# forfd8960/audio-flow-rs

Measured on NVIDIA B200. Metric: audio_seconds_per_second, higher is better.
Workload: dtype f32

## Files before the change

audio-flow-rs_b200/audioflow/__init__.py:

```python
from __future__ import annotations

import ctypes as C
import os
from dataclasses import dataclass
from enum import IntEnum

import numpy as np

_HERE = os.path.dirname(os.path.abspath(__file__))
LIB_PATH = os.environ.get("AF_GPU_LIB") or os.path.join(os.path.dirname(_HERE), "lib", "libaudioflow_gpu.so")

AF_OK, AF_ERR_INVALID, AF_ERR_RESAMPLING_FAILED, AF_ERR_CUDA, AF_ERR_NO_DEVICE, AF_ERR_CAPACITY = range(6)
AF_FMT_F32, AF_FMT_I16 = 0, 1
AF_MEM_DEVICE, AF_MEM_HOST = 0, 1


class AudioError(Exception):
    """src-tauri/src/error.rs:96-111; only ResamplingFailed arises on this path."""


class ResamplingFailed(AudioError):
    def __init__(self, msg: str):
        super().__init__("Resampling failed: " + msg)
        self.msg = msg
# ... 109 lines not shown
        "af_batch_run_host": (C.c_int, [vp, C.POINTER(OutputsC)]),
        "af_pipeline_run": (C.c_int, [vp, C.POINTER(StreamDescC), sz, C.POINTER(OutputsC)]),
        "af_set_kernel_variant": (C.c_int, [C.c_char_p]),
        "af_vad_segments": (C.c_int, [vp, C.c_uint64, vp, sz, vp, C.c_uint32, vp, vp]),
        "af_vad_gate": (C.c_int, [vp, C.c_uint64, vp, C.c_uint64, C.c_uint32, vp, C.c_uint32, vp, C.c_uint32, vp, sz,
                                  C.POINTER(GateOutputsC), vp]),
        "af_current_device": (C.c_int, []), "af_set_stream": (C.c_int, [vp]), "af_init_multi": (C.c_int, [C.c_int]),
        "af_comm_unique_id": (C.c_int, [u8p]), "af_comm_init_rank": (C.c_int, [C.c_int, C.c_int, u8p]),
        "af_comm_size": (C.c_int, []), "af_comm_shutdown": (C.c_int, []),
        "af_shard_partition": (C.c_int, [C.POINTER(StreamDescC), sz, C.c_int, szp]),
        "af_sharded_batch_create": (C.c_int, [vp, C.POINTER(StreamDescC), sz, C.c_int, C.POINTER(vp)]),
        "af_sharded_batch_destroy": (None, [vp]),
        "af_sharded_batch_shard": (C.c_int, [vp, C.c_int, szp, szp, C.POINTER(C.c_int)]),
        "af_sharded_batch_local": (vp, [vp, C.c_int]),
        "af_sharded_batch_run": (C.c_int, [vp, C.POINTER(ShardedOutputsC), C.c_int, C.c_int]),
        "af_sharded_batch_wait": (C.c_int, [vp]), "af_sharded_batch_join": (C.c_int, [vp]),
        "af_sharded_batch_gathered": (C.c_int, [vp, C.c_int, C.POINTER(vp), C.POINTER(C.c_uint64), C.POINTER(C.c_uint64),
                                                C.POINTER(C.c_uint32)]),
        "af_sharded_batch_gathered_host": (C.c_int, [vp, C.c_int, u8p, C.c_uint64]),
        "af_sharded_batch_gather_ms": (C.c_int, [vp, C.c_int, fp]),
        "af_sharded_batch_run_host": (C.c_int, [vp, C.POINTER(OutputsC)]),
        "af_debug_vad_energy_threshold": (C.c_float, [C.c_float]),
        "af_debug_resample_plan": (sz, [C.c_uint32, C.c_uint32, sz, fp, sz, C.POINTER(C.c_int)]),
        "af_session_create": (C.c_int, [vp, sz, C.c_uint32, C.c_uint16, C.c_uint16, C.c_uint32, C.POINTER(vp)]),
        "af_session_destroy": (None, [vp]),
        "af_session_push": (C.c_int, [vp, vp, C.c_uint64, C.c_uint32, C.c_int, C.POINTER(OutputsC),
                                      C.POINTER(C.c_uint32), C.POINTER(C.c_uint32), C.POINTER(C.c_uint32)]),
        "af_session_reset": (C.c_int, [vp]),
        "af_session_enable_levels": (C.c_int, [vp, C.c_int]),
        "af_session_levels": (C.c_int, [vp, fp, fp, u8p]),
        "af_session_enable_wire": (C.c_int, [vp, C.POINTER(WireConfigC)]),
        "af_session_wire": (C.c_int, [vp, C.POINTER(vp), C.POINTER(C.c_uint64), C.POINTER(vp), C.POINTER(C.c_uint64),
                                      C.POINTER(WireTickC), C.POINTER(C.c_uint64)]),
        "af_ring_create": (C.c_int, [sz, C.POINTER(vp)]), "af_ring_destroy": (None, [vp]),
        "af_ring_capacity": (sz, [vp]), "af_ring_write": (sz, [vp, fp, sz]),
        "af_ring_read": (C.c_int, [vp, fp, sz, szp]), "af_ring_available": (sz, [vp]), "af_ring_clear": (None, [vp]),
        "af_session_push_rings": (C.c_int, [vp, C.POINTER(vp), C.c_uint32, C.POINTER(OutputsC),
                                            C.POINTER(C.c_uint32), C.POINTER(C.c_uint32), C.POINTER(C.c_uint32)]),
        "af_session_push_streams": (C.c_int, [vp, vp, C.c_uint64, C.POINTER(C.c_uint32), u8p, C.c_int, C.POINTER(OutputsC),
                                              C.POINTER(C.c_uint32), C.POINTER(C.c_uint32), C.POINTER(C.c_uint32)]),
        "af_session_reset_streams": (C.c_int, [vp, C.POINTER(C.c_uint32), sz]),
        "af_session_push_rings_available": (C.c_int, [vp, C.POINTER(vp), C.c_uint32, u8p, C.POINTER(OutputsC),
                                                      C.POINTER(C.c_uint32), C.POINTER(C.c_uint32), C.POINTER(C.c_uint32)]),
        "af_session_wire_first_frames": (C.c_int, [vp, C.POINTER(C.c_uint64)]),
        "af_session_create_formats": (C.c_int, [vp, sz, C.POINTER(StreamFormatC), sz, C.POINTER(C.c_uint32), C.c_uint16,
                                                C.POINTER(vp)]),
# ... 216 lines not shown
    def energy_db(self) -> float: return float(load_library().af_vad_energy_db(self._h))
    def is_speaking(self) -> bool: return bool(load_library().af_vad_is_speaking(self._h))
    def speech_frame_count(self) -> int: return int(load_library().af_vad_speech_frame_count(self._h))
    def smoothed_energy(self) -> float: return float(load_library().af_vad_smoothed_energy(self._h))


def pcm16_encode(samples) -> np.ndarray:
    x = _f32(samples)
    out = np.empty(len(x), np.int16)
    _check(load_library().af_pcm16_encode(_fp(x), len(x), out.ctypes.data_as(C.POINTER(C.c_int16))))
    return out


def pcm16_base64(samples) -> bytes:
    L = load_library()
    x = _f32(samples)
    cap = int(L.af_pcm16_base64_len(len(x)))
    buf = C.create_string_buffer(max(cap, 1))
    n = C.c_size_t(0)
    _check(L.af_pcm16_base64(_fp(x), len(x), buf, cap, C.byref(n)))
    return buf.raw[:n.value]


def pipeline_config(n_mels: int = 80, vad: VadConfig | None = None, vad_enable: bool = True, vad_frame_len: int = 0,
                    vad_hop: int = 0, write_pcm: bool = True, log10: bool = False, f_min: float = 0.0,
                    f_max: float = 8000.0, log_floor: float = 1e-10, pcm16: bool = False) -> PipelineConfigC:
    c = PipelineConfigC()
    load_library().af_pipeline_config_default(C.byref(c))
    c.n_mels = n_mels
    c.f_min, c.f_max, c.log_floor, c.log10 = f_min, f_max, log_floor, int(log10)
    c.vad_enable = int(vad_enable)
    if vad is not None:
        c.vad = vad._c()
    c.vad_frame_len, c.vad_hop = vad_frame_len, vad_hop
    c.write_pcm = int(write_pcm)
    c.pcm16 = int(pcm16)
    return c


class Pipeline:
    def __init__(self, cfg: PipelineConfigC | None = None):
        self.cfg = cfg if cfg is not None else pipeline_config()
        h = C.c_void_p()
        _check(load_library().af_pipeline_create(C.byref(self.cfg), C.byref(h)))
        self._h = h

    def __del__(self):
        if getattr(self, "_h", None) and _lib is not None:
            _lib.af_pipeline_destroy(self._h)
            self._h = None

    def batch(self, descs, mem: int) -> "Batch":
        return Batch(self, descs, mem)

    def run_host(self, streams):
        arrays, descs = [], []
        for (x, rate, ch) in streams:
            if x.dtype == np.int16:
                a, fmt = np.ascontiguousarray(x), AF_FMT_I16
            else:
                a, fmt = _f32(x), AF_FMT_F32
            arrays.append(a)
            descs.append((a.ctypes.data, a.size, rate, ch, fmt))
        b = Batch(self, descs, AF_MEM_HOST)
        out = b.alloc_host_outputs()
        b.run_host(out)
        return b.split(out)


def _desc_array(descs):
    arr = (StreamDescC * max(len(descs), 1))()
    for i, (ptr, n_samples, rate, ch, fmt) in enumerate(descs):
        arr[i] = StreamDescC(ptr or None, n_samples, rate, ch, fmt)
# ... 399 lines not shown
```

audio-flow-rs_b200/csrc/af_common.cuh:

```cuda
#pragma once
#include <cstddef>
#include <cstdint>
#include <cuda_runtime.h>

namespace af {

constexpr int OUT_RATE = 16000;
constexpr int WIN = 400;
constexpr int HOP = 160;
constexpr int NFFT = 512;
constexpr int NBIN = NFFT / 2 + 1;
constexpr int MAX_MELS = 128;

constexpr int RS_CHUNK = 128;
constexpr int RS_POLY = 8;

constexpr int SF = 32;
constexpr int STEP_SAMPLES = SF * HOP;
constexpr int CARRY = WIN - HOP;
constexpr int YLEN = STEP_SAMPLES + CARRY;
constexpr int N_STAGE = 2;
constexpr int MAX_PARTS = 4;
__host__ __device__ constexpr int part_end(int parts, int k)
{
// ... 172 lines not shown
    int state;
    unsigned long long silence_frames;
    unsigned long long speech_frames;
};

struct FusedParams {
    const StreamDev *streams;
    const TileDev *tiles;
    uint32_t n_tiles;
    const FftTables *fft;
    const MelTables *mel;
    float *pcm;   uint64_t pcm_stride;
    float *logmel; uint64_t logmel_stride;
    float *energy; uint64_t energy_stride;
    uint32_t n_mels;
    uint32_t do_energy;
    float log_floor;
    float log_scale;
    uint32_t use_stage;
    uint32_t layout;
    uint32_t quarters;
    float neg_zero;
    uint32_t per_p, per_q;
};

}
```

audio-flow-rs_b200/csrc/af_fused.cu:

```cuda
#include <atomic>
#include <type_traits>

#ifdef AF_FUSED_SPLIT_TU
#define af_fused_kernel af_fused_split_kernel
#define g_pipe_stats g_pipe_stats_split
#endif

#include "af_device.cuh"
#include "af_launch.h"

namespace af {

constexpr int AF_MAX_GPUS_INTERNAL = 16;

struct alignas(16) RsTile {
    uint32_t stream_idx, tile;
    int tile_k;
    uint32_t tile_rem;
    uint32_t n_steps, tile_end, n_frames, parts;
    StreamDev stream;
    uint32_t inc_k, inc_rem;
};
static_assert(sizeof(RsTile) == 112 && offsetof(RsTile, stream) == 32, "RsTile mirrors the head and the tail of TileDev");
static_assert(offsetof(TileDev, sdesc) % 16 == 0 && sizeof(TileDev) - offsetof(TileDev, sdesc) == 80 && offsetof(TileDev, parts) == 28 &&
              offsetof(TileDev, inc_k) == offsetof(TileDev, sdesc) + sizeof(StreamDev), "TileDev layout the cp.async prefetch relies on");

struct __align__(128) FusedSmem {
    unsigned char stage[N_STAGE][STAGE_BYTES];
    float ybuf[2][YBUF_FLOATS];
    float scr[FFT_WARPS * SCR_FLOATS_PER_WARP];
    float pbuf[2][PBUF_FLOATS];
    uint32_t tmem_base;
// ... 776 lines not shown
    {                                                                                               \
        float w_[16];                                                                               \
        tmem_ld16(tq + 16u * (i), w_);                                                              \
        const float4 xa = pa[i], xb = pb[i], xc = pc[i], xd = pd[i];                                \
        tmem_wait_ld(w_);                                                                           \
        const float4 wa = make_float4(w_[0], w_[1], w_[2], w_[3]), wb = make_float4(w_[4], w_[5], w_[6], w_[7]);       \
        const float4 wc = make_float4(w_[8], w_[9], w_[10], w_[11]), wd = make_float4(w_[12], w_[13], w_[14], w_[15]); \
        AF_MEL_FMA16()                                                                              \
    }
#define AF_MEL_CHAIN(STEP)                                                                          \
    switch (c4) {                                                                                   \
    case 8: STEP(7)                                                                                 \
    case 7: STEP(6)                                                                                 \
    case 6: STEP(5)                                                                                 \
    case 5: STEP(4)                                                                                 \
    case 4: STEP(3)                                                                                 \
    case 3: STEP(2)                                                                                 \
    case 2: STEP(1)                                                                                 \
    case 1: STEP(0)                                                                                 \
    default: break;                                                                                 \
    }

template <bool FAST_LOG, bool VEC>
__device__ __forceinline__ void role_mel_run(FusedSmem &sm, const FusedParams &P, int mw, int lane)
{
    const uint32_t M = P.n_mels;
    const float log_mul = P.log_scale, log_floor = P.log_floor;
    const int q0 = sm.mel.quad_begin[mw], q1 = sm.mel.quad_begin[mw + 1];
    const int fr = pb_frame(lane);
    const uint32_t tm = sm.tmem_base + ((uint32_t)(32 * ((threadIdx.x >> 5) & 3)) << 16);
    AF_STATS_DECL
    for (uint32_t it = 0;; ++it) {
        const int b = (int)(it & 1u);
        AF_WAIT(&sm.p_full[b], (it >> 1) & 1u, 0);
        const StepInfo info = sm.pinfo[it & 3u];
        const int n_valid = info.n_valid & 0xff;
        if (M && info.lm_dst && n_valid > 0) {
            const bool valid = fr < n_valid;
            float *dst = info.lm_dst + (uint32_t)fr * M + 4 * q0;
            const char *prow = reinterpret_cast<const char *>(sm.pbuf[b] + lane * PB_ROW);
            const uint4 *qtab = reinterpret_cast<const uint4 *>(&sm.mel.quad[q0]);
            for (int qd = q0; qd < q1; ++qd, qtab += 2, dst += 4) {
                const uint4 d0q = qtab[0], d1q = qtab[1];
                const float4 *pa = reinterpret_cast<const float4 *>(prow + d0q.x);
                const float4 *pb = reinterpret_cast<const float4 *>(prow + d0q.y);
                const float4 *pc = reinterpret_cast<const float4 *>(prow + d0q.z);
                const float4 *pd = reinterpret_cast<const float4 *>(prow + d0q.w);
                int c4 = (int)d1q.x;
                float a0 = 0.0f, a1 = 0.0f, b0 = 0.0f, b1 = 0.0f, c0 = 0.0f, c1 = 0.0f, d0 = 0.0f, d1 = 0.0f;
                if (d1q.z != MEL_NO_TMEM) {
                    const uint32_t tq = tm + d1q.z;
                    AF_MEL_CHAIN(AF_MEL_STEP_T)
                } else {
                    const float4 *w4 = reinterpret_cast<const float4 *>(reinterpret_cast<const char *>(sm.mel.w) + d1q.y);
#pragma unroll 1
                    for (; c4 > 8; --c4) AF_MEL_STEP_S(c4 - 1)
                    AF_MEL_CHAIN(AF_MEL_STEP_S)
                }
                float o[4];
                if (FAST_LOG) {
                    o[0] = lg2_ftz(fmaxf(a0 + a1, log_floor)) * log_mul;
                    o[1] = lg2_ftz(fmaxf(b0 + b1, log_floor)) * log_mul;
                    o[2] = lg2_ftz(fmaxf(c0 + c1, log_floor)) * log_mul;
                    o[3] = lg2_ftz(fmaxf(d0 + d1, log_floor)) * log_mul;
                } else {
                    o[0] = __log2f(fmaxf(a0 + a1, log_floor)) * log_mul;
                    o[1] = __log2f(fmaxf(b0 + b1, log_floor)) * log_mul;
                    o[2] = __log2f(fmaxf(c0 + c1, log_floor)) * log_mul;
                    o[3] = __log2f(fmaxf(d0 + d1, log_floor)) * log_mul;
                }
                if (valid) {
                    if (VEC) __stcs(reinterpret_cast<float4 *>(dst), make_float4(o[0], o[1], o[2], o[3]));
                    else {
#pragma unroll
                        for (int u = 0; u < 4; ++u)
                            if (4 * qd + u < (int)M) dst[u] = o[u];
                    }
                }
            }
        }
        warp_arrive(&sm.p_empty[b], lane);
        if (info.n_valid & STEP_LAST) break;
    }
    AF_STATS_FLUSH(1, lane);
}
#undef AF_MEL_CHAIN
#undef AF_MEL_STEP_T
#undef AF_MEL_STEP_S
#undef AF_MEL_FMA16

__device__ __forceinline__ void role_mel(FusedSmem &sm, const FusedParams &P, int mw, int lane)
{
    const bool fast_log = P.log_floor >= 1.17549435e-38f;
    const bool vec = (P.n_mels & 3u) == 0 && (P.logmel_stride & 3ull) == 0 && ((reinterpret_cast<uintptr_t>(P.logmel) & 15) == 0);
    if (fast_log && vec) role_mel_run<true, true>(sm, P, mw, lane);
    else if (vec) role_mel_run<false, true>(sm, P, mw, lane);
    else role_mel_run<false, false>(sm, P, mw, lane);
}

template <bool QUARTERS>
__device__ __forceinline__ void role_vad(FusedSmem &sm, const FusedParams &P, int lane, int vidx)
{
    const bool chains = P.do_energy && P.energy;
    if (vidx != 0 && !chains) return;
    AF_STATS_DECL
    uint32_t tile_f = blockIdx.x, g_f = 0, it_f = 0, steps_f = 0;
    int h_f = 0;
    bool fill_live = vidx == 0 && tile_f < P.n_tiles;
    FillDesc d_next{};
    auto fetch_desc = [&]() {
        const uint4 *src = reinterpret_cast<const uint4 *>(&P.tiles[tile_f].fill[2 * g_f + h_f]);
        const uint4 a = __ldg(src), b = __ldg(src + 1);
        d_next.src = reinterpret_cast<const char *>(((unsigned long long)a.y << 32) | a.x);
        d_next.bytes = a.z; d_next.lo = a.w; d_next.hi = b.x; d_next.interior = b.y;
    };
    auto tile_pairs = [&]() { return QUARTERS ? P.tiles[tile_f].n_steps * (P.tiles[tile_f].parts >> 1) : P.tiles[tile_f].n_steps; };
    if (lane == 0 && fill_live) { steps_f = tile_pairs(); fetch_desc(); }
    auto issue_next = [&](bool blocking) {
        if (!fill_live) return;
        if (blocking) { AF_WAIT(&sm.stage_empty[h_f], (it_f & 1u) ^ 1u, 0); }
// ... 426 lines not shown
```

audio-flow-rs_b200/csrc/af_plan.cpp:

```cpp
#include "af_plan.h"

#include <algorithm>
#include <cmath>
#include <cstring>
#include <limits>
#include <numeric>

namespace af {

void RsRecurrence::init(uint32_t in, uint32_t out)
{
    in_rate = in; out_rate = out;
    passthrough = (in == out);
    const uint32_t g = std::gcd(in, out);
    p = in / g; q = out / g;
    const double ratio = (double)out / (double)in;
    t = 1.0 / ratio;
    end_idx = (long)RS_CHUNK - (RS_POLY + 1) - (long)std::ceil(t);
    exact = (q & (q - 1)) == 0 && q <= (1u << 20) && t == (double)p / (double)q;
    last_index = -(double)(RS_POLY / 2);
    chunks = 0; n_out = 0;
}

uint32_t RsRecurrence::step(std::vector<float> *frac)
// ... 103 lines not shown
        cost[qd] = 24u * c4 + 40u;
        total += cost[qd];
    }
    t->n_w = (uint16_t)(16 * off16); t->n_mels = (uint16_t)n_mels;
    uint32_t q = 0, acc = 0;
    t->quad_begin[0] = 0;
    for (int j = 1; j < MEL_WARPS; ++j) {
        const uint32_t target = (uint32_t)(((uint64_t)total * (uint64_t)j) / MEL_WARPS);
        while (q < n_quads && acc + cost[q] / 2 < target) acc += cost[q++];
        t->quad_begin[j] = (uint16_t)q;
    }
    t->quad_begin[MEL_WARPS] = (uint16_t)n_quads;
    uint32_t next_col[4] = {TM_MEL0, TM_MEL0, TM_MEL0, TM_MEL0};
    for (int j = 0; j < MEL_WARPS; ++j) {
        uint32_t &col = next_col[j & 3];
        for (uint32_t qd = t->quad_begin[j]; qd < t->quad_begin[j + 1]; ++qd) {
            const uint32_t need = 16u * t->quad[qd].c4;
            if (t->quad[qd].c4 <= 8 && col + need <= TMEM_COLS) { t->quad[qd].tcol = col; col += need; }
        }
    }
    return true;
}

static inline float bits_to_f32(uint32_t b) { float f; std::memcpy(&f, &b, 4); return f; }

float vad_energy_threshold(float threshold_db)
{
    auto speech = [&](float e) { return 20.0f * log10f(e) > threshold_db; };
    const uint32_t inf_bits = 0x7f800000u;
    if (!speech(bits_to_f32(inf_bits))) return std::numeric_limits<float>::quiet_NaN();
    uint32_t lo = 1, hi = inf_bits;
    if (speech(bits_to_f32(lo))) return bits_to_f32(lo);
    while (hi - lo > 1) {
        const uint32_t mid = lo + (hi - lo) / 2;
        if (speech(bits_to_f32(mid))) hi = mid; else lo = mid;
    }
    return bits_to_f32(hi);
}

}
```

audio-flow-rs_b200/csrc/af_plan.h:

```cpp
#pragma once
#include <cstdint>
#include <vector>

#include "af_common.cuh"

namespace af {

struct RsRecurrence {
    uint32_t in_rate = 0, out_rate = 0;
    uint32_t p = 1, q = 1;
    double t = 1.0;
    long end_idx = 0;
    bool passthrough = false;
    bool exact = false;
    double last_index = -4.0;
    uint64_t chunks = 0;
    uint64_t n_out = 0;

    void init(uint32_t in, uint32_t out);
    uint32_t step(std::vector<float> *frac);
    uint32_t mode() const { return passthrough ? RS_PASSTHROUGH : (exact ? RS_EXACT : RS_TABLE); }
};

uint64_t rs_exact_count(const RsRecurrence &r, uint64_t chunks);

void build_fft_tables(FftTables *t);
bool build_mel_tables(uint32_t n_mels, float f_min, float f_max, MelTables *t);
float vad_energy_threshold(float threshold_db);

}
```

audio-flow-rs_b200/csrc/af_runtime.cu:

```cuda
#include <algorithm>
#include <cmath>
#include <cstdlib>
#include <cstring>

#include "af_internal.h"

using namespace af;
using namespace afrt;

namespace afrt {

namespace {
thread_local std::string g_err;
std::atomic<uint64_t> g_launches{0};
Context *const g_ctxs = new Context[MAX_DEV];
std::mutex g_init_mu;
std::atomic<int> g_default_dev{-1};
thread_local int t_dev = -1;
std::string g_variant = "auto";
}

int fail(int code, const char *fmt, ...)
{
    char buf[512];
    va_list ap;
    va_start(ap, fmt);
    vsnprintf(buf, sizeof(buf), fmt, ap);
    va_end(ap);
// ... 662 lines not shown
    cudaStream_t st = cuda_stream ? (cudaStream_t)cuda_stream : cur_ctx().stream;
    GateJob J{};
    J.pcm = out->pcm ? pcm : nullptr; J.pcm_stride = pcm_stride;
    J.logmel = out->logmel ? logmel : nullptr; J.logmel_stride = logmel_stride;
    J.n_mels = n_mels; J.hop = hop; J.n_out = n_out;
    J.seg = seg; J.seg_cap = seg_cap; J.n_seg = n_seg;
    J.off = out->seg_offset; J.total = out->n_frames;
    J.out_pcm = out->pcm; J.out_pcm_stride = out->pcm_stride;
    J.out_lm = out->logmel; J.out_lm_stride = out->logmel_stride;
    J.n_streams = (uint32_t)n_streams;
    AF_CUDA(launch_vad_gate(J, st));
    count_launch((J.out_pcm || J.out_lm) ? 2 : 1);
    if (!cuda_stream) AF_CUDA(cudaStreamSynchronize(st));
    return AF_OK;
}

}

struct af_pipeline {
    af_pipeline_config cfg;
    VadParams vad_prm;
    MelTables h_mel;
    DevBuf<MelTables> d_mel[MAX_DEV];
    std::mutex mu;
};

namespace {
MelTables *pipe_mel(af_pipeline *p)
{
    if (!p->cfg.n_mels) return nullptr;
    const int dev = cur_device();
    std::lock_guard<std::mutex> lk(p->mu);
    if (!p->d_mel[dev].get()) {
        cudaError_t e = p->d_mel[dev].alloc(1);
        if (e == cudaSuccess) e = cudaMemcpy(p->d_mel[dev].get(), &p->h_mel, sizeof(MelTables), cudaMemcpyHostToDevice);
        if (e != cudaSuccess) {
            p->d_mel[dev].reset();
            fail(AF_ERR_CUDA, "mel tables: %s", cudaGetErrorString(e));
        }
    }
    return p->d_mel[dev].get();
}
}

namespace {

struct HostStream {
    af_stream_desc desc;
    uint32_t n_in, n_out, n_frames, n_vad_frames, mode, p, q;
    std::shared_ptr<FracTable> table;
// ... 95 lines not shown
int run_sub(af_batch *b, SubBatch &sb, float *pcm, uint64_t pcm_stride, float *logmel, uint64_t logmel_stride,
            uint8_t *vad, uint64_t vad_stride, float *energy, uint64_t energy_stride, VadState *vad_final,
            cudaStream_t st)
{
    const af_pipeline_config &cfg = b->pipe->cfg;
    const bool stft_vad = cfg.vad_enable && cfg.vad_frame_len == 0;
    const bool custom_vad = cfg.vad_enable && cfg.vad_frame_len != 0;
    if (!sb.h_tiles.empty()) {
        FusedParams P{};
        P.streams = sb.d_streams.get(); P.tiles = sb.d_tiles.get(); P.n_tiles = (uint32_t)sb.h_tiles.size();
        P.fft = cur_ctx().d_fft.get(); P.mel = b->d_mel;
        P.pcm = pcm; P.pcm_stride = pcm_stride;
        P.logmel = cfg.n_mels ? logmel : nullptr; P.logmel_stride = logmel_stride;
        P.energy = stft_vad ? energy : nullptr; P.energy_stride = energy_stride;
        P.n_mels = (cfg.n_mels && logmel) ? cfg.n_mels : 0;
        P.do_energy = stft_vad ? 1 : 0;
        P.log_floor = cfg.log_floor;
        P.log_scale = cfg.log10 ? 0.30102999566398120f : 0.69314718055994531f;
        P.use_stage = kernel_variant() == "sync" ? 0u : 1u;
        P.layout = fused_layout(stft_vad);
        P.quarters = sb.quarters ? 1u : 0u;
        P.neg_zero = -0.0f;
        P.per_p = sb.per_p; P.per_q = sb.per_q;
        const int n_ctas = (int)std::min<size_t>(sb.h_tiles.size(), (size_t)cur_ctx().sm_count);
        AF_CUDA(launch_fused(P, n_ctas, st, sb.split));
        count_launch();
    }
    if (custom_vad) {
        EnergyJob ej{};
        ej.y = pcm; ej.y_stride = pcm_stride; ej.n_frames = sb.d_nvad.get(); ej.n_frames_all = (uint32_t)b->max_vad;
        ej.frame_len = cfg.vad_frame_len; ej.hop = cfg.vad_hop; ej.energy = energy; ej.energy_stride = energy_stride;
        ej.n_streams = (uint32_t)sb.count;
        AF_CUDA(launch_frame_energy(ej, st));
        count_launch();
    }
    if (cfg.vad_enable) {
        ScanJob sj{};
        sj.energy = energy; sj.energy_stride = energy_stride; sj.n_frames = sb.d_nvad.get(); sj.n_frames_all = 0;
        sj.states = vad; sj.states_stride = vad_stride; sj.state_io = nullptr; sj.final_out = vad_final;
        sj.prm = b->pipe->vad_prm; sj.n_streams = (uint32_t)sb.count;
        if (b->max_vad > 16384 && b->max_vad < 0x40000000ull) {
            AF_CUDA(sb.d_scan.grow(sb.count * scan_scratch_words((uint32_t)b->max_vad)));
            sj.max_frames = (uint32_t)b->max_vad; sj.scratch = sb.d_scan.get();
        }
        AF_CUDA(launch_vad_scan(sj, st));
        count_launch();
// ... 19 lines not shown
    cfg->log10 = 0;
    cfg->vad_enable = 1;
    af_vad_config_default(&cfg->vad);
    cfg->vad_frame_len = 0; cfg->vad_hop = 0;
    cfg->write_pcm = 1;
    cfg->pcm16 = 0;
}

AF_API int af_pipeline_create(const af_pipeline_config *cfg, af_pipeline **out)
{
    if (!out) return fail(AF_ERR_INVALID, "null out pointer");
    int rc = require_ctx();
    if (rc) return rc;
    af_pipeline_config c;
    if (cfg) c = *cfg; else af_pipeline_config_default(&c);
    if (c.n_mels > MAX_MELS) return fail(AF_ERR_INVALID, "n_mels %u > %d", c.n_mels, MAX_MELS);
    if (c.vad_enable && c.vad_frame_len != 0 && c.vad_hop == 0) return fail(AF_ERR_INVALID, "vad_hop must be positive");
    if (c.n_mels && !(c.f_max > c.f_min && c.f_min >= 0.0f)) return fail(AF_ERR_INVALID, "bad mel band [%g, %g]", c.f_min, c.f_max);
    af_pipeline *p = new af_pipeline;
    p->cfg = c;
    p->vad_prm = make_vad_params(c.vad);
    if (c.n_mels) {
        if (!build_mel_tables(c.n_mels, c.f_min, c.f_max, &p->h_mel)) { delete p; return fail(AF_ERR_INVALID, "mel table construction failed"); }
        if (!pipe_mel(p)) { delete p; return AF_ERR_CUDA; }
    }
    *out = p;
    return AF_OK;
}

AF_API void af_pipeline_destroy(af_pipeline *p)
{
    if (!p) return;
    for (int d = 0; d < MAX_DEV; ++d)
        if (p->d_mel[d].get() && device_ctx(d)) { DevScope scope_(d); p->d_mel[d].reset(); }
    delete p;
}

AF_API void af_batch_destroy(af_batch *b)
{
    if (!b) return;
    DevScope scope_(b->device);
    cudaDeviceSynchronize();
    for (auto &s : b->slots)
        if (s.st) cudaStreamDestroy(s.st);
    delete b;
}
// ... 277 lines not shown
            if (o->energy)
                AF_CUDA(cudaMemcpy2DAsync(o->energy + r0 * o->energy_stride, o->energy_stride * sizeof(float), sl.d_energy.get(),
                                          b->energy_stride * sizeof(float), b->max_vad * sizeof(float), sb.count,
                                          cudaMemcpyDeviceToHost, st));
        }
        if (cfg.vad_enable && o->vad_final)
            AF_CUDA(cudaMemcpyAsync(o->vad_final + r0, sl.d_final.get(), sb.count * sizeof(VadState), cudaMemcpyDeviceToHost, st));
    }
    for (auto &sl : b->slots) AF_CUDA(cudaStreamSynchronize(sl.st));
    return AF_OK;
}

AF_API int af_pipeline_run(af_pipeline *p, const af_stream_desc *streams, size_t n_streams, const af_outputs *out)
{
    af_batch *b = nullptr;
    int rc = af_batch_create(p, streams, n_streams, AF_MEM_HOST, &b);
    if (rc) return rc;
    rc = af_batch_run_host(b, out);
    af_batch_destroy(b);
    return rc;
}

AF_API float af_debug_vad_energy_threshold(float threshold_db) { return vad_energy_threshold(threshold_db); }

AF_API size_t af_debug_resample_plan(uint32_t input_rate, uint32_t output_rate, size_t n_chunks, float *frac, size_t cap,
                                     int *mode)
{
    RsRecurrence r;
    r.init(input_rate, output_rate);
    if (mode) *mode = (int)r.mode();
    if (r.passthrough || r.end_idx <= 0) return 0;
    std::vector<float> f;
    for (size_t c = 0; c < n_chunks; ++c) r.step(&f);
    for (size_t i = 0; i < f.size() && i < cap; ++i) frac[i] = f[i];
    return f.size();
}

}

struct af_session {
    af_pipeline *pipe = nullptr;
    int device = -1;
    MelTables *d_mel = nullptr;
    size_t S = 0;
    struct Format { uint32_t rate, channels, max_tick_frames; };
    std::vector<Format> fmts;
// ... 449 lines not shown
        AF_CUDA(cudaMemcpy2DAsync(o->pcm, o->pcm_stride * sizeof(float), pcm_rows, pcm_rows_stride * sizeof(float),
                                  (size_t)max_ny * sizeof(float), S, cudaMemcpyDeviceToHost, st));
    if (s->levels) {
        AF_CUDA(launch_peak(ycur + one.y_keep, s->y_stride, one.n_y, (uint32_t)S, s->lv.d_peak.get(), st, tab));
        count_launch();
    }

    if (maxT) {
        if (s->packed) {
            FusedParams P{};
            P.streams = s->d_ptab[y_next].get(); P.tiles = s->d_ptiles[y_next].get(); P.n_tiles = s->pk_n;
            const uint64_t vrows = s->pk_rows;
            P.fft = cur_ctx().d_fft.get(); P.mel = s->d_mel;
            P.pcm = nullptr; P.pcm_stride = 0;
            P.logmel = lm; P.logmel_stride = lm_stride * vrows;
            P.energy = cfg.vad_enable ? s->d_energy.get() : nullptr; P.energy_stride = s->energy_stride * vrows;
            P.n_mels = lm ? cfg.n_mels : 0;
            P.do_energy = cfg.vad_enable ? 1 : 0;
            P.log_floor = cfg.log_floor;
            P.log_scale = cfg.log10 ? 0.30102999566398120f : 0.69314718055994531f;
            P.use_stage = kernel_variant() == "sync" ? 0u : 1u;
            P.layout = fused_layout(P.do_energy != 0);
            P.neg_zero = -0.0f;
            if (P.n_mels || P.do_energy) {
                AF_CUDA(launch_fused(P, (int)std::min<size_t>(P.n_tiles, (size_t)cur_ctx().sm_count), st));
                count_launch(2);
            }
        } else {
            EnergyJob ej{};
            ej.y = ycur; ej.y_stride = s->y_stride; ej.n_frames = d_T; ej.n_frames_all = maxT;
            ej.frame_len = s->frame_len; ej.hop = s->hop; ej.energy = s->d_energy.get(); ej.energy_stride = s->energy_stride;
            ej.n_streams = (uint32_t)S;
            AF_CUDA(launch_frame_energy(ej, st));
            count_launch();
        }
        if (cfg.vad_enable) {
            ScanJob sj{};
            sj.energy = s->d_energy.get(); sj.energy_stride = s->energy_stride; sj.n_frames = d_T; sj.n_frames_all = maxT;
            sj.states = states; sj.states_stride = st_stride; sj.state_io = s->d_vad.get();
            sj.final_out = mem == AF_MEM_DEVICE ? reinterpret_cast<VadState *>(o->vad_final) : nullptr;
            sj.prm = s->pipe->vad_prm; sj.n_streams = (uint32_t)S;
            AF_CUDA(launch_vad_scan(sj, st));
            count_launch();
        }
        if (mem == AF_MEM_DEVICE && lm && lm != o->logmel)
            AF_CUDA(cudaMemcpy2DAsync(o->logmel, o->logmel_stride * sizeof(float), lm, lm_stride * sizeof(float),
// ... 373 lines not shown
```

include/audioflow_gpu.h:

```cpp
#ifndef AUDIOFLOW_GPU_H
#define AUDIOFLOW_GPU_H

#include <stddef.h>
#include <stdint.h>

#ifdef __cplusplus
extern "C" {
#endif

#if defined(__GNUC__)
#define AF_API __attribute__((visibility("default")))
#else
#define AF_API
#endif

typedef enum af_status {
    AF_OK = 0,
    AF_ERR_INVALID = 1,
    AF_ERR_RESAMPLING_FAILED = 2,
    AF_ERR_CUDA = 3,
    AF_ERR_NO_DEVICE = 4,
    AF_ERR_CAPACITY = 5
} af_status;

// ... 152 lines not shown
AF_API int af_shard_partition(const af_stream_desc *streams, size_t n_streams, int n_shards, size_t *first);

typedef struct af_sharded_batch af_sharded_batch;
typedef struct af_sharded_outputs {
    af_outputs shard[AF_MAX_GPUS];
} af_sharded_outputs;
AF_API int af_sharded_batch_create(af_pipeline *p, const af_stream_desc *streams, size_t n_streams, int mem,
                                   af_sharded_batch **out);
AF_API void af_sharded_batch_destroy(af_sharded_batch *b);
AF_API int af_sharded_batch_shard(const af_sharded_batch *b, int rank, size_t *first, size_t *count, int *device);
AF_API af_batch *af_sharded_batch_local(af_sharded_batch *b, int rank);
AF_API int af_sharded_batch_run(af_sharded_batch *b, const af_sharded_outputs *out, int gather, int async);
AF_API int af_sharded_batch_wait(af_sharded_batch *b);
AF_API int af_sharded_batch_join(af_sharded_batch *b);
AF_API int af_sharded_batch_gathered(af_sharded_batch *b, int rank, const uint8_t **states, uint64_t *row_stride,
                                     uint64_t *rows_per_rank, uint32_t *n_vad_frames);
AF_API int af_sharded_batch_gathered_host(af_sharded_batch *b, int rank, uint8_t *states, uint64_t stride);
AF_API int af_sharded_batch_gather_ms(af_sharded_batch *b, int rank, float *ms);
AF_API int af_sharded_batch_run_host(af_sharded_batch *b, const af_outputs *out);

AF_API float af_debug_vad_energy_threshold(float threshold_db);
AF_API size_t af_debug_resample_plan(uint32_t input_rate, uint32_t output_rate, size_t n_chunks, float *frac,
                                     size_t cap, int *mode);

typedef struct af_session af_session;
AF_API int af_session_create(af_pipeline *p, size_t n_streams, uint32_t sample_rate, uint16_t channels,
                             uint16_t format, uint32_t max_tick_samples, af_session **out);
AF_API void af_session_destroy(af_session *s);
AF_API int af_session_push(af_session *s, const void *data, uint64_t in_stride, uint32_t n_samples, int mem,
                           const af_outputs *out, uint32_t *n_pcm, uint32_t *n_feat, uint32_t *n_vad);
AF_API int af_session_reset(af_session *s);

AF_API int af_session_enable_levels(af_session *s, int enable);
AF_API int af_session_levels(const af_session *s, float *level_db, float *peak, uint8_t *is_speech);

typedef struct af_wire_config {
    uint32_t gate;
    uint32_t pcm16;
    uint32_t base64;
    int32_t mem;
} af_wire_config;
typedef struct af_wire_tick {
    uint32_t n_samples, n_chars, continued;
    uint16_t started, ended;
    uint8_t in_speech, pad[3];
} af_wire_tick;
// ... 39 lines not shown
```

Measured before the change: 13.51 million.

## Specialize mel filterbank for common configs with generated unrolled FMA walks

```diff
diff --git a/audio-flow-rs_b200/audioflow/__init__.py b/audio-flow-rs_b200/audioflow/__init__.py
--- a/audio-flow-rs_b200/audioflow/__init__.py
+++ b/audio-flow-rs_b200/audioflow/__init__.py
@@ -155,6 +155,8 @@
         "af_sharded_batch_run_host": (C.c_int, [vp, C.POINTER(OutputsC)]),
         "af_debug_vad_energy_threshold": (C.c_float, [C.c_float]),
         "af_debug_resample_plan": (sz, [C.c_uint32, C.c_uint32, sz, fp, sz, C.POINTER(C.c_int)]),
+        "af_debug_mel_bank": (C.c_int, [C.c_uint32, C.c_float, C.c_float, fp, fp, C.POINTER(C.c_uint32)]),
+        "af_debug_pipeline_mel_bank": (C.c_int, [vp]),
         "af_session_create": (C.c_int, [vp, sz, C.c_uint32, C.c_uint16, C.c_uint16, C.c_uint32, C.POINTER(vp)]),
         "af_session_destroy": (None, [vp]),
         "af_session_push": (C.c_int, [vp, vp, C.c_uint64, C.c_uint32, C.c_int, C.POINTER(OutputsC),
@@ -417,6 +419,18 @@
     return buf.raw[:n.value]
 
 
+def mel_bank(n_mels: int, f_min: float = 0.0, f_max: float = 8000.0) -> dict:
+    L = load_library()
+    plan = np.zeros((n_mels, 257), np.float32)
+    comp = np.full((n_mels, 257), np.nan, np.float32)
+    wb = (C.c_uint32 * 5)(*([0xFFFFFFFF] * 5))
+    bank = L.af_debug_mel_bank(n_mels, f_min, f_max, _fp(plan), _fp(comp), wb)
+    if bank < 0:
+        raise ValueError(f"no mel filterbank for n_mels={n_mels}, [{f_min}, {f_max}] Hz")
+    has = wb[0] != 0xFFFFFFFF
+    return {"bank": bank, "plan": plan, "compiled": comp if has else None, "warp_bands": list(wb) if has else None}
+
+
 def pipeline_config(n_mels: int = 80, vad: VadConfig | None = None, vad_enable: bool = True, vad_frame_len: int = 0,
                     vad_hop: int = 0, write_pcm: bool = True, log10: bool = False, f_min: float = 0.0,
                     f_max: float = 8000.0, log_floor: float = 1e-10, pcm16: bool = False) -> PipelineConfigC:
@@ -444,6 +458,10 @@
         if getattr(self, "_h", None) and _lib is not None:
             _lib.af_pipeline_destroy(self._h)
             self._h = None
+
+    @property
+    def mel_bank(self) -> int:
+        return int(load_library().af_debug_pipeline_mel_bank(self._h))
 
     def batch(self, descs, mem: int) -> "Batch":
         return Batch(self, descs, mem)
diff --git a/audio-flow-rs_b200/csrc/af_common.cuh b/audio-flow-rs_b200/csrc/af_common.cuh
--- a/audio-flow-rs_b200/csrc/af_common.cuh
+++ b/audio-flow-rs_b200/csrc/af_common.cuh
@@ -218,6 +218,7 @@
     uint32_t quarters;
     float neg_zero;
     uint32_t per_p, per_q;
-};
-
-}
+    uint32_t mel_bank;
+};
+
+}
diff --git a/audio-flow-rs_b200/csrc/af_fused.cu b/audio-flow-rs_b200/csrc/af_fused.cu
--- a/audio-flow-rs_b200/csrc/af_fused.cu
+++ b/audio-flow-rs_b200/csrc/af_fused.cu
@@ -8,6 +8,7 @@
 
 #include "af_device.cuh"
 #include "af_launch.h"
+#include "af_mel_banks.h"
 
 namespace af {
 
@@ -830,6 +831,32 @@
     }
 
 template <bool FAST_LOG, bool VEC>
+__device__ __forceinline__ void mel_out4(float *dst, int m0, uint32_t M, bool valid, float log_floor, float log_mul, float s0,
+                                         float s1, float s2, float s3)
+{
+    float o[4];
+    if (FAST_LOG) {
+        o[0] = lg2_ftz(fmaxf(s0, log_floor)) * log_mul;
+        o[1] = lg2_ftz(fmaxf(s1, log_floor)) * log_mul;
+        o[2] = lg2_ftz(fmaxf(s2, log_floor)) * log_mul;
+        o[3] = lg2_ftz(fmaxf(s3, log_floor)) * log_mul;
+    } else {
+        o[0] = __log2f(fmaxf(s0, log_floor)) * log_mul;
+        o[1] = __log2f(fmaxf(s1, log_floor)) * log_mul;
+        o[2] = __log2f(fmaxf(s2, log_floor)) * log_mul;
+        o[3] = __log2f(fmaxf(s3, log_floor)) * log_mul;
+    }
+    if (valid) {
+        if (VEC) __stcs(reinterpret_cast<float4 *>(dst), make_float4(o[0], o[1], o[2], o[3]));
+        else {
+#pragma unroll
+            for (int u = 0; u < 4; ++u)
+                if (m0 + u < (int)M) dst[u] = o[u];
+        }
+    }
+}
+
+template <int BANK, bool FAST_LOG, bool VEC>
 __device__ __forceinline__ void role_mel_run(FusedSmem &sm, const FusedParams &P, int mw, int lane)
 {
     const uint32_t M = P.n_mels;
@@ -845,45 +872,34 @@
         const int n_valid = info.n_valid & 0xff;
         if (M && info.lm_dst && n_valid > 0) {
             const bool valid = fr < n_valid;
-            float *dst = info.lm_dst + (uint32_t)fr * M + 4 * q0;
-            const char *prow = reinterpret_cast<const char *>(sm.pbuf[b] + lane * PB_ROW);
-            const uint4 *qtab = reinterpret_cast<const uint4 *>(&sm.mel.quad[q0]);
-            for (int qd = q0; qd < q1; ++qd, qtab += 2, dst += 4) {
-                const uint4 d0q = qtab[0], d1q = qtab[1];
-                const float4 *pa = reinterpret_cast<const float4 *>(prow + d0q.x);
-                const float4 *pb = reinterpret_cast<const float4 *>(prow + d0q.y);
-                const float4 *pc = reinterpret_cast<const float4 *>(prow + d0q.z);
-                const float4 *pd = reinterpret_cast<const float4 *>(prow + d0q.w);
-                int c4 = (int)d1q.x;
-                float a0 = 0.0f, a1 = 0.0f, b0 = 0.0f, b1 = 0.0f, c0 = 0.0f, c1 = 0.0f, d0 = 0.0f, d1 = 0.0f;
-                if (d1q.z != MEL_NO_TMEM) {
-                    const uint32_t tq = tm + d1q.z;
-                    AF_MEL_CHAIN(AF_MEL_STEP_T)
-                } else {
-                    const float4 *w4 = reinterpret_cast<const float4 *>(reinterpret_cast<const char *>(sm.mel.w) + d1q.y);
+            if constexpr (BANK != 0) {
+                float *dst = info.lm_dst + (uint32_t)fr * M;
+                auto emit = [&](int m0, float s0, float s1, float s2, float s3) {
+                    mel_out4<FAST_LOG, VEC>(dst + m0, m0, M, valid, log_floor, log_mul, s0, s1, s2, s3);
+                };
+                mel_bank_walk<BANK>(mw, reinterpret_cast<const float4 *>(sm.pbuf[b] + lane * PB_ROW), emit);
+            } else {
+                float *dst = info.lm_dst + (uint32_t)fr * M + 4 * q0;
+                const char *prow = reinterpret_cast<const char *>(sm.pbuf[b] + lane * PB_ROW);
+                const uint4 *qtab = reinterpret_cast<const uint4 *>(&sm.mel.quad[q0]);
+                for (int qd = q0; qd < q1; ++qd, qtab += 2, dst += 4) {
+                    const uint4 d0q = qtab[0], d1q = qtab[1];
+                    const float4 *pa = reinterpret_cast<const float4 *>(prow + d0q.x);
+                    const float4 *pb = reinterpret_cast<const float4 *>(prow + d0q.y);
+                    const float4 *pc = reinterpret_cast<const float4 *>(prow + d0q.z);
+                    const float4 *pd = reinterpret_cast<const float4 *>(prow + d0q.w);
+                    int c4 = (int)d1q.x;
+                    float a0 = 0.0f, a1 = 0.0f, b0 = 0.0f, b1 = 0.0f, c0 = 0.0f, c1 = 0.0f, d0 = 0.0f, d1 = 0.0f;
+                    if (d1q.z != MEL_NO_TMEM) {
+                        const uint32_t tq = tm + d1q.z;
+                        AF_MEL_CHAIN(AF_MEL_STEP_T)
+                    } else {
+                        const float4 *w4 = reinterpret_cast<const float4 *>(reinterpret_cast<const char *>(sm.mel.w) + d1q.y);
 #pragma unroll 1
-                    for (; c4 > 8; --c4) AF_MEL_STEP_S(c4 - 1)
-                    AF_MEL_CHAIN(AF_MEL_STEP_S)
-                }
-                float o[4];
-                if (FAST_LOG) {
-                    o[0] = lg2_ftz(fmaxf(a0 + a1, log_floor)) * log_mul;
-                    o[1] = lg2_ftz(fmaxf(b0 + b1, log_floor)) * log_mul;
-                    o[2] = lg2_ftz(fmaxf(c0 + c1, log_floor)) * log_mul;
-                    o[3] = lg2_ftz(fmaxf(d0 + d1, log_floor)) * log_mul;
-                } else {
-                    o[0] = __log2f(fmaxf(a0 + a1, log_floor)) * log_mul;
-                    o[1] = __log2f(fmaxf(b0 + b1, log_floor)) * log_mul;
-                    o[2] = __log2f(fmaxf(c0 + c1, log_floor)) * log_mul;
-                    o[3] = __log2f(fmaxf(d0 + d1, log_floor)) * log_mul;
-                }
-                if (valid) {
-                    if (VEC) __stcs(reinterpret_cast<float4 *>(dst), make_float4(o[0], o[1], o[2], o[3]));
-                    else {
-#pragma unroll
-                        for (int u = 0; u < 4; ++u)
-                            if (4 * qd + u < (int)M) dst[u] = o[u];
+                        for (; c4 > 8; --c4) AF_MEL_STEP_S(c4 - 1)
+                        AF_MEL_CHAIN(AF_MEL_STEP_S)
                     }
+                    mel_out4<FAST_LOG, VEC>(dst, 4 * qd, M, valid, log_floor, log_mul, a0 + a1, b0 + b1, c0 + c1, d0 + d1);
                 }
             }
         }
@@ -897,13 +913,21 @@
 #undef AF_MEL_STEP_S
 #undef AF_MEL_FMA16
 
-__device__ __forceinline__ void role_mel(FusedSmem &sm, const FusedParams &P, int mw, int lane)
+template <int BANK>
+__device__ __forceinline__ void role_mel_bank(FusedSmem &sm, const FusedParams &P, int mw, int lane)
 {
     const bool fast_log = P.log_floor >= 1.17549435e-38f;
     const bool vec = (P.n_mels & 3u) == 0 && (P.logmel_stride & 3ull) == 0 && ((reinterpret_cast<uintptr_t>(P.logmel) & 15) == 0);
-    if (fast_log && vec) role_mel_run<true, true>(sm, P, mw, lane);
-    else if (vec) role_mel_run<false, true>(sm, P, mw, lane);
-    else role_mel_run<false, false>(sm, P, mw, lane);
+    if (fast_log && vec) role_mel_run<BANK, true, true>(sm, P, mw, lane);
+    else if (vec) role_mel_run<BANK, false, true>(sm, P, mw, lane);
+    else role_mel_run<BANK, false, false>(sm, P, mw, lane);
+}
+static_assert(N_MEL_BANKS == 2, "role_mel dispatches on every compiled filterbank");
+__device__ __forceinline__ void role_mel(FusedSmem &sm, const FusedParams &P, int mw, int lane)
+{
+    if (P.mel_bank == 1u) role_mel_bank<1>(sm, P, mw, lane);
+    else if (P.mel_bank == 2u) role_mel_bank<2>(sm, P, mw, lane);
+    else role_mel_bank<0>(sm, P, mw, lane);
 }
 
 template <bool QUARTERS>
diff --git a/audio-flow-rs_b200/csrc/af_plan.cpp b/audio-flow-rs_b200/csrc/af_plan.cpp
--- a/audio-flow-rs_b200/csrc/af_plan.cpp
+++ b/audio-flow-rs_b200/csrc/af_plan.cpp
@@ -149,6 +149,15 @@
     return true;
 }
 
+void mel_dense_row(const MelTables &t, uint32_t m, float row[NBIN])
+{
+    std::memset(row, 0, sizeof(float) * NBIN);
+    const MelQuad &Q = t.quad[m / 4];
+    const uint32_t u = m & 3u, first = Q.off[u] / 4u, woff16 = Q.woff / 64u;
+    for (uint32_t k = 0; k < 4u * Q.c4; ++k)
+        if (first + k < (uint32_t)NBIN) row[first + k] = t.w[16u * (woff16 + k / 4u) + 4u * u + (k & 3u)];
+}
+
 static inline float bits_to_f32(uint32_t b) { float f; std::memcpy(&f, &b, 4); return f; }
 
 float vad_energy_threshold(float threshold_db)
diff --git a/audio-flow-rs_b200/csrc/af_plan.h b/audio-flow-rs_b200/csrc/af_plan.h
--- a/audio-flow-rs_b200/csrc/af_plan.h
+++ b/audio-flow-rs_b200/csrc/af_plan.h
@@ -26,6 +26,15 @@
 
 void build_fft_tables(FftTables *t);
 bool build_mel_tables(uint32_t n_mels, float f_min, float f_max, MelTables *t);
+void mel_dense_row(const MelTables &t, uint32_t m, float row[NBIN]);
+
+struct MelBank {
+    uint32_t n_mels;
+    float f_min, f_max;
+    uint16_t band_begin[MEL_WARPS + 1];
+    const uint16_t *lo, *n, *off;
+    const float *w;
+};
 float vad_energy_threshold(float threshold_db);
 
 }
diff --git a/audio-flow-rs_b200/csrc/af_runtime.cu b/audio-flow-rs_b200/csrc/af_runtime.cu
--- a/audio-flow-rs_b200/csrc/af_runtime.cu
+++ b/audio-flow-rs_b200/csrc/af_runtime.cu
@@ -4,6 +4,7 @@
 #include <cstring>
 
 #include "af_internal.h"
+#include "af_mel_banks.h"
 
 using namespace af;
 using namespace afrt;
@@ -712,10 +713,28 @@
     VadParams vad_prm;
     MelTables h_mel;
     DevBuf<MelTables> d_mel[MAX_DEV];
+    uint32_t mel_bank = 0;
     std::mutex mu;
 };
 
 namespace {
+uint32_t mel_bank_for(uint32_t n_mels, float f_min, float f_max, const MelTables &t)
+{
+    for (int i = 0; i < N_MEL_BANKS; ++i) {
+        const MelBank &B = MEL_BANKS[i];
+        if (B.n_mels != n_mels || B.f_min != f_min || B.f_max != f_max) continue;
+        bool same = true;
+        for (uint32_t m = 0; m < n_mels && same; ++m) {
+            float row[NBIN], bank[NBIN] = {};
+            mel_dense_row(t, m, row);
+            memcpy(bank + B.lo[m], B.w + B.off[m], sizeof(float) * B.n[m]);
+            same = memcmp(row, bank, sizeof(row)) == 0;
+        }
+        if (same) return (uint32_t)i + 1;
+    }
+    return 0;
+}
+
 MelTables *pipe_mel(af_pipeline *p)
 {
     if (!p->cfg.n_mels) return nullptr;
@@ -857,6 +876,7 @@
         P.quarters = sb.quarters ? 1u : 0u;
         P.neg_zero = -0.0f;
         P.per_p = sb.per_p; P.per_q = sb.per_q;
+        P.mel_bank = b->pipe->mel_bank;
         const int n_ctas = (int)std::min<size_t>(sb.h_tiles.size(), (size_t)cur_ctx().sm_count);
         AF_CUDA(launch_fused(P, n_ctas, st, sb.split));
         count_launch();
@@ -922,6 +942,7 @@
     p->vad_prm = make_vad_params(c.vad);
     if (c.n_mels) {
         if (!build_mel_tables(c.n_mels, c.f_min, c.f_max, &p->h_mel)) { delete p; return fail(AF_ERR_INVALID, "mel table construction failed"); }
+        p->mel_bank = mel_bank_for(c.n_mels, c.f_min, c.f_max, p->h_mel);
         if (!pipe_mel(p)) { delete p; return AF_ERR_CUDA; }
     }
     *out = p;
@@ -1245,6 +1266,27 @@
 }
 
 AF_API float af_debug_vad_energy_threshold(float threshold_db) { return vad_energy_threshold(threshold_db); }
+
+AF_API int af_debug_mel_bank(uint32_t n_mels, float f_min, float f_max, float *plan_w, float *bank_w, uint32_t *warp_bands)
+{
+    MelTables t;
+    if (!build_mel_tables(n_mels, f_min, f_max, &t)) return -1;
+    if (plan_w)
+        for (uint32_t m = 0; m < n_mels; ++m) mel_dense_row(t, m, plan_w + (size_t)m * NBIN);
+    for (int i = 0; i < N_MEL_BANKS; ++i) {
+        const MelBank &B = MEL_BANKS[i];
+        if (B.n_mels != n_mels || B.f_min != f_min || B.f_max != f_max) continue;
+        for (uint32_t m = 0; bank_w && m < n_mels; ++m) {
+            float *row = bank_w + (size_t)m * NBIN;
+            std::fill(row, row + NBIN, 0.0f);
+            memcpy(row + B.lo[m], B.w + B.off[m], sizeof(float) * B.n[m]);
+        }
+        for (int j = 0; warp_bands && j <= MEL_WARPS; ++j) warp_bands[j] = B.band_begin[j];
+    }
+    return (int)mel_bank_for(n_mels, f_min, f_max, t);
+}
+
+AF_API int af_debug_pipeline_mel_bank(const af_pipeline *p) { return p ? (int)p->mel_bank : -1; }
 
 AF_API size_t af_debug_resample_plan(uint32_t input_rate, uint32_t output_rate, size_t n_chunks, float *frac, size_t cap,
                                      int *mode)
@@ -1740,6 +1782,7 @@
             P.use_stage = kernel_variant() == "sync" ? 0u : 1u;
             P.layout = fused_layout(P.do_energy != 0);
             P.neg_zero = -0.0f;
+            P.mel_bank = s->pipe->mel_bank;
             if (P.n_mels || P.do_energy) {
                 AF_CUDA(launch_fused(P, (int)std::min<size_t>(P.n_tiles, (size_t)cur_ctx().sm_count), st));
                 count_launch(2);
diff --git a/audio-flow-rs_b200/csrc/gen_mel_banks.cpp b/audio-flow-rs_b200/csrc/gen_mel_banks.cpp
--- /dev/null
+++ b/audio-flow-rs_b200/csrc/gen_mel_banks.cpp
@@ -0,0 +1,179 @@
+#include <cstdio>
+#include <cstring>
+#include <string>
+#include <vector>
+
+#include "af_plan.h"
+
+using namespace af;
+
+namespace {
+
+struct BankCfg { uint32_t n_mels; float f_min, f_max; const char *what; };
+const BankCfg BANKS[] = {{80, 0.0f, 8000.0f, "HTK, 80 bands, 0-8000 Hz"}, {128, 0.0f, 8000.0f, "HTK, 128 bands, 0-8000 Hz"}};
+constexpr int N_BANKS = sizeof(BANKS) / sizeof(BANKS[0]);
+
+std::string hexf(float v)
+{
+    char b[64];
+    std::snprintf(b, sizeof(b), "%af", (double)v);
+    return b;
+}
+
+struct Filter { int lo = 0, hi = 0; };
+
+struct Bank {
+    BankCfg cfg;
+    std::vector<std::vector<float>> dense;
+    std::vector<Filter> f;
+    uint16_t band_begin[MEL_WARPS + 1];
+};
+
+long warp_cost(const Bank &B, int b0, int b1)
+{
+    long nnz = 0, gmin = 1 << 30, gmax = -1;
+    for (int m = b0; m < b1; ++m) {
+        for (int k = 0; k < NBIN; ++k) nnz += B.dense[m][k] != 0.0f;
+        if (B.f[m].hi > B.f[m].lo) { gmin = std::min<long>(gmin, B.f[m].lo / 4); gmax = std::max<long>(gmax, (B.f[m].hi - 1) / 4); }
+    }
+    return nnz + (gmax >= gmin ? gmax - gmin + 1 : 0) + 4 * (b1 - b0);
+}
+
+void split(Bank &B)
+{
+    const int nq = (int)(B.cfg.n_mels + 3) / 4, M = (int)B.cfg.n_mels;
+    auto band = [&](int q) { return std::min(4 * q, M); };
+    long best = -1;
+    for (int c1 = 0; c1 <= nq; ++c1)
+        for (int c2 = c1; c2 <= nq; ++c2)
+            for (int c3 = c2; c3 <= nq; ++c3) {
+                const int cut[MEL_WARPS + 1] = {0, c1, c2, c3, nq};
+                long worst = 0;
+                for (int j = 0; j < MEL_WARPS; ++j) worst = std::max(worst, warp_cost(B, band(cut[j]), band(cut[j + 1])));
+                if (best < 0 || worst < best) {
+                    best = worst;
+                    for (int j = 0; j <= MEL_WARPS; ++j) B.band_begin[j] = (uint16_t)band(cut[j]);
+                }
+            }
+}
+
+void emit_walk(FILE *o, const Bank &B, int id, int j)
+{
+    const int b0 = B.band_begin[j], b1 = B.band_begin[j + 1];
+    int gmin = 1 << 30, gmax = -1, nnz = 0;
+    for (int m = b0; m < b1; ++m)
+        if (B.f[m].hi > B.f[m].lo) { gmin = std::min(gmin, B.f[m].lo / 4); gmax = std::max(gmax, (B.f[m].hi - 1) / 4); }
+    for (int m = b0; m < b1; ++m)
+        for (int k = 0; k < NBIN; ++k) nnz += B.dense[m][k] != 0.0f;
+    std::fprintf(o, "// bank %d, mel warp %d: bands [%d, %d), %d LDS.128, %d FFMA\n", id, j, b0, b1, gmax >= gmin ? gmax - gmin + 1 : 0, nnz);
+    std::fprintf(o, "template <class Emit>\n__device__ __forceinline__ void mel_walk_%d_%d(const float4 *__restrict__ r, Emit &emit)\n{\n", id, j);
+    for (int m = b0; m < b1; ++m)
+        if (B.f[m].hi > B.f[m].lo) std::fprintf(o, "    float e%d = 0.0f, o%d = 0.0f;\n", m, m);
+    auto sum = [&](int m) -> std::string {
+        if (m >= (int)B.cfg.n_mels || B.f[m].hi <= B.f[m].lo) return "0.0f";
+        bool odd = false;
+        for (int k = B.f[m].lo; k < B.f[m].hi; ++k) odd |= (k & 1) && B.dense[m][k] != 0.0f;
+        return odd ? "e" + std::to_string(m) + " + o" + std::to_string(m) : "e" + std::to_string(m);
+    };
+    auto done_at = [&](int q) {
+        int g = 1 << 30;
+        for (int m = q; m < q + 4 && m < b1; ++m)
+            if (B.f[m].hi > B.f[m].lo) g = std::min(g, B.f[m].lo / 4);
+        return g == (1 << 30) ? -1 : g;
+    };
+    auto emit_quad = [&](int q) {
+        std::fprintf(o, "    emit(%d, %s, %s, %s, %s);\n", q, sum(q).c_str(), sum(q + 1).c_str(), sum(q + 2).c_str(), sum(q + 3).c_str());
+    };
+    for (int q = b0; q < b1; q += 4)
+        if (done_at(q) < 0) emit_quad(q);
+    static const char comp[4] = {'x', 'y', 'z', 'w'};
+    static const int order[4] = {0, 2, 1, 3};
+    for (int g = gmax; g >= gmin; --g) {
+        std::fprintf(o, "    {\n        const float4 x = r[%d];\n", g);
+        for (int m = b0; m < b1; ++m)
+            for (int c : order) {
+                const int k = 4 * g + c;
+                if (k >= NBIN || B.dense[m][k] == 0.0f) continue;
+                const char acc = (c & 1) ? 'o' : 'e';
+                std::fprintf(o, "        %c%d = fmaf(%s, x.%c, %c%d);\n", acc, m, hexf(B.dense[m][k]).c_str(), comp[c], acc, m);
+            }
+        std::fprintf(o, "    }\n");
+        for (int q = b0; q < b1; q += 4)
+            if (done_at(q) == g) emit_quad(q);
+    }
+    std::fprintf(o, "}\n\n");
+}
+
+}
+
+int main(int argc, char **argv)
+{
+    if (argc != 2) { std::fprintf(stderr, "usage: %s OUT.h\n", argv[0]); return 2; }
+    std::vector<Bank> banks;
+    for (const BankCfg &c : BANKS) {
+        Bank B;
+        B.cfg = c;
+        static MelTables t;
+        if (!build_mel_tables(c.n_mels, c.f_min, c.f_max, &t)) { std::fprintf(stderr, "build_mel_tables failed for %s\n", c.what); return 1; }
+        B.dense.assign(c.n_mels, std::vector<float>(NBIN, 0.0f));
+        B.f.resize(c.n_mels);
+        for (uint32_t m = 0; m < c.n_mels; ++m) {
+            mel_dense_row(t, m, B.dense[m].data());
+            int lo = -1, hi = 0;
+            for (int k = 0; k < NBIN; ++k)
+                if (B.dense[m][k] != 0.0f) { if (lo < 0) lo = k; hi = k + 1; }
+            B.f[m] = lo < 0 ? Filter{} : Filter{lo, hi};
+        }
+        split(B);
+        banks.push_back(B);
+    }
+
+    FILE *o = std::fopen(argv[1], "w");
+    if (!o) { std::perror(argv[1]); return 1; }
+    std::fprintf(o, "// af_mel_banks.h -- written by gen_mel_banks (csrc/gen_mel_banks.cpp) from build_mel_tables at build time.\n"
+                    "#pragma once\n#include \"af_plan.h\"\n\nnamespace af {\n\n");
+    std::fprintf(o, "constexpr int N_MEL_BANKS = %d;      // bank ids 1 .. N_MEL_BANKS; 0 = the generic quad path\n\n", N_BANKS);
+    for (int i = 0; i < N_BANKS; ++i) {
+        const Bank &B = banks[i];
+        const int id = i + 1, M = (int)B.cfg.n_mels;
+        std::vector<float> w;
+        std::vector<int> off;
+        for (int m = 0; m < M; ++m) {
+            off.push_back((int)w.size());
+            for (int k = B.f[m].lo; k < B.f[m].hi; ++k) w.push_back(B.dense[m][k]);
+        }
+        std::fprintf(o, "// bank %d: %s (%zu weights in the filters' spans)\n", id, B.cfg.what, w.size());
+        const char *names[3] = {"lo", "n", "off"};
+        for (int a = 0; a < 3; ++a) {
+            std::fprintf(o, "inline constexpr uint16_t mel_bank%d_%s[%d] = {", id, names[a], M);
+            for (int m = 0; m < M; ++m)
+                std::fprintf(o, "%s%d", m ? ", " : "", a == 0 ? B.f[m].lo : (a == 1 ? B.f[m].hi - B.f[m].lo : off[m]));
+            std::fprintf(o, "};\n");
+        }
+        std::fprintf(o, "inline constexpr float mel_bank%d_w[%zu] = {", id, w.size() ? w.size() : 1);
+        for (size_t k = 0; k < w.size(); ++k) std::fprintf(o, "%s%s%s", k ? "," : "", k % 6 == 0 ? "\n    " : " ", hexf(w[k]).c_str());
+        std::fprintf(o, "};\n\n");
+    }
+    std::fprintf(o, "inline constexpr MelBank MEL_BANKS[N_MEL_BANKS] = {\n");
+    for (int i = 0; i < N_BANKS; ++i) {
+        const Bank &B = banks[i];
+        std::fprintf(o, "    {%u, %s, %s, {", B.cfg.n_mels, hexf(B.cfg.f_min).c_str(), hexf(B.cfg.f_max).c_str());
+        for (int j = 0; j <= MEL_WARPS; ++j) std::fprintf(o, "%s%u", j ? ", " : "", B.band_begin[j]);
+        std::fprintf(o, "}, mel_bank%d_lo, mel_bank%d_n, mel_bank%d_off, mel_bank%d_w},\n", i + 1, i + 1, i + 1, i + 1);
+    }
+    std::fprintf(o, "};\n\n#ifdef __CUDACC__\n");
+    for (int i = 0; i < N_BANKS; ++i)
+        for (int j = 0; j < MEL_WARPS; ++j) emit_walk(o, banks[i], i + 1, j);
+    std::fprintf(o, "// mel warp mw's share of bank BANK for the frame whose power row is r\n"
+                    "template <int BANK, class Emit>\n"
+                    "__device__ __forceinline__ void mel_bank_walk(int mw, const float4 *__restrict__ r, Emit &emit)\n{\n");
+    for (int i = 0; i < N_BANKS; ++i) {
+        std::fprintf(o, "    %sif constexpr (BANK == %d) {\n", i ? "else " : "", i + 1);
+        for (int j = 0; j < MEL_WARPS; ++j)
+            std::fprintf(o, "        %sif (mw == %d) mel_walk_%d_%d(r, emit);\n", j ? "else " : "", j, i + 1, j);
+        std::fprintf(o, "    }\n");
+    }
+    std::fprintf(o, "}\n#endif\n\n}  // namespace af\n");
+    if (std::fclose(o) != 0) { std::perror(argv[1]); return 1; }
+    return 0;
+}
diff --git a/include/audioflow_gpu.h b/include/audioflow_gpu.h
--- a/include/audioflow_gpu.h
+++ b/include/audioflow_gpu.h
@@ -198,6 +198,8 @@
 AF_API float af_debug_vad_energy_threshold(float threshold_db);
 AF_API size_t af_debug_resample_plan(uint32_t input_rate, uint32_t output_rate, size_t n_chunks, float *frac,
                                      size_t cap, int *mode);
+AF_API int af_debug_mel_bank(uint32_t n_mels, float f_min, float f_max, float *plan_w, float *bank_w, uint32_t *warp_bands);
+AF_API int af_debug_pipeline_mel_bank(const af_pipeline *p);
 
 typedef struct af_session af_session;
 AF_API int af_session_create(af_pipeline *p, size_t n_streams, uint32_t sample_rate, uint16_t channels,
```

Result: slower. 12.26 million, median of 6 (-9.2%).
